# syghmon/bridges-with-reinforcement-learning

Measured on AMD Instinct MI355X. Metric: env-steps/sec (vectorised assembly_gym, tower_height=4), higher is better.
Workload: dtype f64

## Files before the change

bridges-with-reinforcement-learning_amd/csrc/api.hip:

```cpp
#include <hip/hip_runtime.h>
#include <cstdio>
#include <cstdlib>
#include <cstring>
#include <new>

#include "env_kernels.hip"
#include "ops_kernels.hip"
#include "dqn_kernels.hip"
#include "mlp_kernels.hip"
#include "conv_kernels.hip"
#include "conv_train_kernels.hip"

using namespace bridges;

static thread_local char g_err[512] = "";

static int fail_hip(hipError_t e, const char* what) {
    snprintf(g_err, sizeof(g_err), "%s: %s", what, hipGetErrorString(e));
    return BRIDGES_E_HIP;
}
static int fail_arg(const char* what) {
    snprintf(g_err, sizeof(g_err), "bad argument: %s", what);
    return BRIDGES_E_ARG;
}
#define HIP_TRY(x)                                        \
    do {                                                  \
        hipError_t e_ = (x);                              \
        if (e_ != hipSuccess) return fail_hip(e_, #x);    \
    } while (0)

template <typename... P, typename... A>
static int launch(const char* name, void (*k)(P...), dim3 grid, dim3 block, size_t lds, void* stream, A... a) {
    hipLaunchKernelGGL(k, grid, block, lds, (hipStream_t)stream, a...);
    const hipError_t e = hipGetLastError();
    return e == hipSuccess ? BRIDGES_OK : fail_hip(e, name);
}

template <typename... T>
static bool aligned(uintptr_t bytes, const T*... p) {
    return ((((uintptr_t)p) | ... | (uintptr_t)0) & (bytes - 1)) == 0;
}

static int64_t ceil_div(int64_t a, int64_t b) { return (a + b - 1) / b; }

static int64_t clamp_grid(int64_t blocks, int64_t limit) {
    if (blocks < 1) blocks = 1;
    return blocks > limit ? limit : blocks;
}

static int grid_for_waves(int64_t n_items) { return (int)clamp_grid(ceil_div(n_items, 4), 2048); }

static int up2_splits(int64_t tiles, int* tps) {
    int per = (int)((tiles + 255) / 256);
    if (per < 1) per = 1;
    *tps = per;
    return (int)((tiles + per - 1) / per);
}

typedef void (*c3_fn)(const float*, const float*, const float*, const float*, const float*, float*, int, int, int, int, int);
template <int W, int CH>
static c3_fn c3_epilogue(int mode) {
    if (mode == C3_EPI_BIAS_RELU) return k_c3<W, CH, C3_EPI_BIAS_RELU>;
    if (mode == C3_EPI_MASK) return k_c3<W, CH, C3_EPI_MASK>;
    return k_c3<W, CH, C3_EPI_RAW>;
}
template <int W>
static c3_fn c3_kernel(int c_in, int mode) { return c_in <= 4 ? c3_epilogue<W, 4>(mode) : c3_epilogue<W, 16>(mode); }

struct bridges_gate {
    hipEvent_t last;
};

struct bridges_env {
    bridges_gate* gate;
    hipEvent_t raster_done;
    DevCtx ctx;
    TaskTable* tt_dev;
    int32_t* h_total;
    int max_blocks;
    int max_faces;
    hipEvent_t* ev_start;
    hipEvent_t* ev_stop;
    int ev_cap, ev_used;
    bool has_tasks;
    bridges_task_buffers tasks;
    const float* fixed_reward_map;
    const double* fixed_reward_prefix;
};

static long long candidate_estimate(const bridges_env* env) {
    long long est = (long long)(*(volatile int32_t*)env->h_total);
    if (est < env->ctx.E) est = env->ctx.E;
    return est + est / 32 + 64;
}

extern "C" {

const char* bridges_last_error(void) { return g_err; }

#ifndef BRIDGES_SRC_HASH
#define BRIDGES_SRC_HASH "unstamped"
#endif
const char* bridges_source_hash(void) { return "BRIDGES_SRC_HASH=" BRIDGES_SRC_HASH; }

int bridges_device_count(void) {
    int n = 0;
    if (hipGetDeviceCount(&n) != hipSuccess) return 0;
    return n;
}

int bridges_env_create(const bridges_task* t, const bridges_env_buffers* buf, bridges_env** out) {
    if (!t || !buf || !out) return fail_arg("null");
    if (t->n_envs <= 0) return fail_arg("n_envs");
    if (t->max_blocks <= 0 || t->max_blocks > BRIDGES_MAX_BLOCKS) return fail_arg("max_blocks > BRIDGES_MAX_BLOCKS");
    if (t->n_shapes <= 0 || t->n_shapes > 8) return fail_arg("n_shapes");
    if (t->n_groups <= 0 || t->n_groups > BRIDGES_MAX_GROUPS) return fail_arg("n_groups");
    if (t->n_ground < 0 || t->n_ground > 32 || t->n_offsets <= 0 || t->n_offsets > 8) return fail_arg("n_ground/n_offsets");
    if (t->n_targets < 0 || t->n_targets > BRIDGES_MAX_TARGETS) return fail_arg("n_targets");
    if (t->a_max <= 0) return fail_arg("a_max");
    if (t->img_size != 0 && (t->img_size < 2 || t->img_size > BRIDGES_IMG)) return fail_arg("img_size must be 0 (= 64) or 2..64");
    if (t->debug != 0) return fail_arg("debug must be 0");
    if (!buf->reward_prefix) return fail_arg("reward_prefix (float64 row prefix sums of reward_map) not given");
    if (buf->lp_ws_stride < (int64_t)BRIDGES_LP_WS_DOUBLES) return fail_arg("lp_ws_stride < BRIDGES_LP_WS_DOUBLES");
    static_assert(BRIDGES_LP_WS_DOUBLES == WARM_WS_DOUBLES, "header and device code disagree on the persistent tableau size");
    static_assert(BRIDGES_LP_SNAP_DOUBLES == WARM_HDR_DOUBLES + WARM_HALF, "header and device code disagree on the snapshot size");
    if (buf->lp_snap && buf->lp_snap_stride < (int64_t)BRIDGES_LP_SNAP_DOUBLES) return fail_arg("lp_snap_stride < BRIDGES_LP_SNAP_DOUBLES");
    for (int g = 0; g < t->n_groups; ++g) {
        if (t->group_shape[g] < 0 || t->group_shape[g] >= t->n_shapes) return fail_arg("group_shape");
        if (t->group_face[g] < 0 || t->group_face[g] >= t->shapes[t->group_shape[g]].nv) return fail_arg("group_face");
    }
    for (int s = 0; s < t->n_shapes; ++s)
        if (t->shapes[s].nv < 3 || t->shapes[s].nv > BRIDGES_MAX_VERTS) return fail_arg("shape nv");
    int ndev = 0;
    if (hipGetDeviceCount(&ndev) != hipSuccess || ndev == 0) {
        snprintf(g_err, sizeof(g_err), "no HIP device");
        return BRIDGES_E_NODEV;
    }
    bridges_env* env = new (std::nothrow) bridges_env();
    if (!env) return fail_arg("oom");
    TaskTable* host = new (std::nothrow) TaskTable();
    if (!host) { delete env; return fail_arg("oom"); }
    memset(host, 0, sizeof(TaskTable));
    memcpy(host->shapes, t->shapes, sizeof(bridges_shape) * t->n_shapes);
    memcpy(host->x_ground, t->x_ground, sizeof(double) * t->n_ground);
    memcpy(host->offsets, t->offsets, sizeof(double) * t->n_offsets);
    const int img = t->img_size ? t->img_size : IMG;
    for (int i = 0; i < IMG; ++i) {
        host->grid_x[i] = t->grid_x[i < img ? i : img - 1];
        host->grid_y[i] = t->grid_y[i < img ? i : img - 1];
    }
    hipError_t e = hipMalloc((void**)&env->tt_dev, sizeof(TaskTable));
    if (e == hipSuccess) e = hipMemcpy(env->tt_dev, host, sizeof(TaskTable), hipMemcpyHostToDevice);
    delete host;
    if (e != hipSuccess) { delete env; return fail_hip(e, "task table upload"); }
    DevCtx& c = env->ctx;
    memset(&c, 0, sizeof(c));
    c.b = *buf;
    c.tt = env->tt_dev;
    c.E = t->n_envs; c.K = t->max_blocks; c.max_steps = t->max_steps; c.a_max = t->a_max;
    c.n_groups = t->n_groups; c.n_ground = t->n_ground; c.n_offsets = t->n_offsets; c.n_targets = t->n_targets;
    memcpy(c.group_shape, t->group_shape, sizeof(c.group_shape));
    memcpy(c.group_face, t->group_face, sizeof(c.group_face));
    c.mu = t->mu; c.density = t->density; c.floor_hw = t->floor_half_width; c.floor_depth = t->floor_depth;
    c.xlim0 = t->xlim[0]; c.xlim1 = t->xlim[1]; c.ylim0 = t->ylim[0]; c.ylim1 = t->ylim[1];
    memcpy(c.targets, t->targets, sizeof(c.targets));
    c.seed = t->seed;
    c.debug = t->debug;
    c.env_id_base = t->env_id_base;
    c.n_shapes = t->n_shapes;
    c.img = img;
    env->ev_start = env->ev_stop = nullptr;
    env->ev_cap = env->ev_used = 0;
    env->gate = nullptr;
    env->raster_done = nullptr;
    env->has_tasks = false;
    memset(&env->tasks, 0, sizeof(env->tasks));
// ... 20 lines not shown
    }
    delete[] env->ev_start;
    delete[] env->ev_stop;
    env->ev_start = env->ev_stop = nullptr;
    env->ev_cap = env->ev_used = 0;
}

int bridges_env_destroy(bridges_env* env) {
    if (!env) return BRIDGES_OK;
    free_events(env);
    if (env->raster_done) (void)hipEventDestroy(env->raster_done);
    (void)hipFree(env->tt_dev);
    (void)hipHostFree(env->h_total);
    delete env;
    return BRIDGES_OK;
}

int bridges_gate_create(bridges_gate** out) {
    if (!out) return fail_arg("gate_create");
    bridges_gate* g = new (std::nothrow) bridges_gate();
    if (!g) return fail_arg("oom");
    g->last = nullptr;
    *out = g;
    return BRIDGES_OK;
}

int bridges_gate_destroy(bridges_gate* gate) {
    delete gate;
    return BRIDGES_OK;
}

int bridges_env_set_gate(bridges_env* env, bridges_gate* gate) {
    if (!env) return fail_arg("set_gate");
    if (gate && !env->raster_done) HIP_TRY(hipEventCreateWithFlags(&env->raster_done, hipEventDisableTiming));
    env->gate = gate;
    return BRIDGES_OK;
}

int bridges_env_timing_begin(bridges_env* env, int32_t max_launches) {
    if (!env || max_launches <= 0 || max_launches > (1 << 16)) return fail_arg("timing_begin");
    free_events(env);
    env->ev_start = new (std::nothrow) hipEvent_t[max_launches];
    env->ev_stop = new (std::nothrow) hipEvent_t[max_launches];
    if (!env->ev_start || !env->ev_stop) {
        delete[] env->ev_start;
        delete[] env->ev_stop;
        env->ev_start = env->ev_stop = nullptr;
        return fail_arg("oom");
    }
    for (int i = 0; i < max_launches; ++i) {
        HIP_TRY(hipEventCreate(&env->ev_start[i]));
        HIP_TRY(hipEventCreate(&env->ev_stop[i]));
        env->ev_cap = i + 1;
    }
    env->ev_used = 0;
    return BRIDGES_OK;
}

int bridges_env_timing_end(bridges_env* env, double* raster_ms_total, int32_t* n_launches) {
    if (!env || !raster_ms_total || !n_launches) return fail_arg("timing_end");
    double total = 0.0;
    for (int i = 0; i < env->ev_used; ++i) {
        HIP_TRY(hipEventSynchronize(env->ev_stop[i]));
        float ms = 0.f;
        HIP_TRY(hipEventElapsedTime(&ms, env->ev_start[i], env->ev_stop[i]));
        total += ms;
    }
    *raster_ms_total = total;
    *n_launches = env->ev_used;
    free_events(env);
    return BRIDGES_OK;
}

static int refresh(bridges_env* env, hipStream_t s, int after_step) {
    const DevCtx& c = env->ctx;
    if (int rc = launch("k_scan", k_scan, dim3(1), dim3(SCAN_THREADS), 0, s, c, after_step)) return rc;
    if (int rc = launch("k_enumerate", k_enumerate, dim3(c.E), dim3(WAVE), 0, s, c)) return rc;
    const long long items_est = candidate_estimate(env) + c.E;
    long long rblocks = ceil_div(items_est, 4);
    if (rblocks > env->max_blocks) rblocks = env->max_blocks;
    const bool timed = env->ev_cap > 0 && env->ev_used < env->ev_cap;
    if (env->gate && env->gate->last) HIP_TRY(hipStreamWaitEvent(s, env->gate->last, 0));
    if (timed) HIP_TRY(hipEventRecord(env->ev_start[env->ev_used], s));
    if (!env->has_tasks) {
        if (int rc = launch("k_raster", env->max_faces <= 4 ? k_raster<4> : k_raster<MAXV>, dim3((unsigned)rblocks), dim3(256), 0, s, c))
            return rc;
    } else if (int rc = launch("k_raster (per-env tables)", env->max_faces <= 4 ? k_raster<4, true> : k_raster<MAXV, true>,
                               dim3((unsigned)rblocks), dim3(256), 0, s, c)) {
        return rc;
    }
    if (timed) { HIP_TRY(hipEventRecord(env->ev_stop[env->ev_used], s)); env->ev_used++; }
    if (env->gate) {
        HIP_TRY(hipEventRecord(env->raster_done, s));
        env->gate->last = env->raster_done;
    }
    return launch("k_select", k_select, dim3(c.E), dim3(WAVE), 0, s, c, 0);
}

static int task_features(bridges_env* env, void* stream, int mode) {
    return launch("k_task_features", k_task_features, dim3(env->ctx.E), dim3(TASK_THREADS), 0, stream, env->ctx, env->tasks, mode);
}

int bridges_env_reset(bridges_env* env, void* stream) {
    if (!env) return fail_arg("null env");
    if (int rc = launch("k_reset", k_reset, dim3(env->ctx.E), dim3(WAVE), 0, stream, env->ctx)) return rc;
    if (env->has_tasks)
        if (int rc = task_features(env, stream, TASK_RESET)) return rc;
    return refresh(env, (hipStream_t)stream, 0);
}

int bridges_env_step(bridges_env* env, void* stream) {
    if (!env) return fail_arg("null env");
    if (!env->has_tasks) {
        if (int rc = launch("k_step", k_step<>, dim3(env->ctx.E), dim3(WAVE), 0, stream, env->ctx)) return rc;
    } else {
        if (int rc = launch("k_step (per-env targets)", k_step<const double*>, dim3(env->ctx.E), dim3(WAVE), 0, stream, env->ctx,
                            (const double*)env->tasks.env_targets))
            return rc;
        if (env->tasks.sample)
            if (int rc = task_features(env, stream, TASK_STEP)) return rc;
    }
    return refresh(env, (hipStream_t)stream, 1);
}

int bridges_env_set_task_buffers(bridges_env* env, const bridges_task_buffers* tb) {
    if (!env) return fail_arg("null env");
    DevCtx& c = env->ctx;
    if (!tb) {
        env->has_tasks = false;
        memset(&env->tasks, 0, sizeof(env->tasks));
        c.b.reward_map = env->fixed_reward_map;
        c.b.reward_prefix = env->fixed_reward_prefix;
        return BRIDGES_OK;
    }
    if (!tb->env_targets || !tb->target_bits || !tb->reward_map || !tb->reward_prefix || !tb->task_episode || !tb->gauss_k)
        return fail_arg("task buffers: env_targets / target_bits / reward_map / reward_prefix / task_episode / gauss_k not given");
    if (tb->env_obstacle_bits) return fail_arg("task buffers: env_obstacle_bits is reserved (obstacles are shared by all envs)");
    if (c.n_targets < 1) return fail_arg("task buffers: the task has no targets");
    if (tb->target_shape < 0 || tb->target_shape >= c.n_shapes) return fail_arg("task buffers: target_shape");
    if (tb->sample != 0 && tb->sample != 1) return fail_arg("task buffers: sample must be 0 or 1");
    if (tb->sample && !(tb->x_range[0] <= tb->x_range[1] && tb->z_range[0] <= tb->z_range[1])) return fail_arg("task buffers: x_range / z_range");
    env->tasks = *tb;
    env->has_tasks = true;
    c.b.reward_map = tb->reward_map;
    c.b.reward_prefix = tb->reward_prefix;
    return BRIDGES_OK;
}

int bridges_env_load_targets(bridges_env* env, void* stream) {
    if (!env) return fail_arg("null env");
    if (!env->has_tasks) return fail_arg("bridges_env_load_targets: no task buffers attached");
    return task_features(env, stream, TASK_LOAD);
}

int bridges_env_refresh(bridges_env* env, void* stream) {
    if (!env) return fail_arg("null env");
    return refresh(env, (hipStream_t)stream, 0);
}

#define CS_TAB_SMALL 768
#define CS_COLS_SMALL 92
#define CS_TAB_LARGE 4096
int bridges_env_candidate_stability(bridges_env* env, void* stream) {
    if (!env) return fail_arg("null env");
    const DevCtx& c = env->ctx;
    if (!c.b.cand_stable || !c.b.cand_queue || !c.b.cand_counters || !c.b.cand_ws) return fail_arg("cand_stable / cand_queue / cand_counters / cand_ws not given");
    if (c.b.cand_ws_stride < (int64_t)(3 * c.K + 2) * (4 * BRIDGES_MAX_INTERFACES + 3)) return fail_arg("cand_ws_stride");
    hipStream_t s = (hipStream_t)stream;
    HIP_TRY(hipMemsetAsync(c.b.cand_counters, 0, 2 * sizeof(int32_t), s));
    long long est = candidate_estimate(env);
    if (est > env->max_blocks) est = env->max_blocks;
    if (int rc = launch("k_candidate_stability", k_candidate_stability<CS_TAB_SMALL, CS_COLS_SMALL, false>, dim3((unsigned)est),
                        dim3(WAVE), 0, s, c))
// ... 820 lines not shown
```

bridges-with-reinforcement-learning_amd/csrc/env_kernels.hip:

```cpp
#include "bridges_device.h"
#include "rbe_device.h"

namespace bridges {

__device__ inline void reset_env(const DevCtx& c, int e, int lane) {
    c.b.state_bits[(size_t)e * IMG + lane] = 0ull;
    if (lane < c.K) c.b.blk_occ[(size_t)e * c.K + lane] = 0;
    if (lane == 0) {
        c.b.n_blocks[e] = 0;
        c.b.n_if[e] = 0;
        c.b.targets_left[e] = (c.n_targets >= 32) ? 0xffffffffu : ((1u << c.n_targets) - 1u);
        c.b.needs_reset[e] = 0;
    }
}

__device__ inline int count_candidates(const DevCtx& c, int e, int nb, int lane) {
    int nfree = 0;
    for (int i0 = 0; i0 < nb * MAXV; i0 += WAVE) {
        int i = i0 + lane;
        bool fr = false;
        if (i < nb * MAXV) {
            int b = i / MAXV, f = i % MAXV;
            int nv = c.tt->shapes[c.b.blk_shape[(size_t)e * c.K + b]].nv;
            fr = f < nv && !((c.b.blk_occ[(size_t)e * c.K + b] >> f) & 1);
// ... 426 lines not shown
                rot2(sn.vx[i], sn.vz[i], cs, sn_, rx, rz);
                wx[i] = px + rx; wz[i] = pz + rz;
                if (wx[i] < c.xlim0 - eps || wx[i] > c.xlim1 + eps || wz[i] < c.ylim0 - eps || wz[i] > c.ylim1 + eps) inb = false;
                if (wz[i] < -eps) inb = false;
            }
            c.b.cand_verts[ci * MAXV * 2 + 2 * i] = wx[i];
            c.b.cand_verts[ci * MAXV * 2 + 2 * i + 1] = wz[i];
        }
        {
#define PICK6(v, k) ((k) == 5 ? v[5] : (k) == 4 ? v[4] : (k) == 3 ? v[3] : (k) == 2 ? v[2] : (k) == 1 ? v[1] : v[0])
#pragma unroll
            for (int f = 0; f < MAXV; ++f) {
                double o0 = 0.0, o1 = 0.0, o2 = 0.0, o3 = 0.0;
                if (f < sn.nv) {
                    const int ia = sn.fa[f], ib = sn.fb[f];
                    const double ax = PICK6(wx, ia), az = PICK6(wz, ia), bx = PICK6(wx, ib), bz = PICK6(wz, ib);
                    Frame2 fr = edge_frame(ax, az, bx, bz);
                    o0 = fr.cx; o1 = fr.cz; o2 = fr.nx; o3 = fr.nz;
                }
                double2* dst = reinterpret_cast<double2*>(c.b.cand_frames + (ci * MAXV + f) * 4);
                dst[0] = make_double2(o0, o1);
                dst[1] = make_double2(o2, o3);
            }
#undef PICK6
            c.b.cand_rows[ci * 2 + 0] = (sn.nv << 16) | ((inb ? 1 : 0) << 24);
            c.b.cand_rows[ci * 2 + 1] = e;
        }
        c.b.cand_pose[ci * 4 + 0] = px; c.b.cand_pose[ci * 4 + 1] = pz;
        c.b.cand_pose[ci * 4 + 2] = cs; c.b.cand_pose[ci * 4 + 3] = sn_;
        c.b.cand_desc[ci * 4 + 0] = tb; c.b.cand_desc[ci * 4 + 1] = tf;
        c.b.cand_desc[ci * 4 + 2] = sh; c.b.cand_desc[ci * 4 + 3] = fc;
        c.b.cand_ox[ci] = ox;
        c.b.cand_inb[ci] = inb;
        c.b.cand_env[ci] = e;
    }
}

__device__ __forceinline__ void write_f32_image(float* img, uint64_t rowbits, int lane, int32_t* nz = nullptr) {
    const int sub = lane >> 4, col4 = (lane & 15) * 4;
    const uint64_t nonzero_rows = __ballot(rowbits != 0ull);
    if (nz) {
        uint64_t t = nonzero_rows | (nonzero_rows >> 1);
        t = (t | (t >> 2)) & 0x1111111111111111ull;
        uint32_t now = 0u;
#pragma unroll
        for (int g = 0; g < IMG / 4; ++g) now |= (uint32_t)((t >> (4 * g)) & 1ull) << g;
        uint32_t need = (uint32_t)__builtin_amdgcn_readfirstlane(*nz) | now;
        if (lane == 0) *nz = (int32_t)now;
        while (need) {
            const int g = __builtin_ctz(need);
            need &= need - 1u;
            uint32_t nib = 0u;
            if ((now >> g) & 1u) {
                uint64_t m = shfl_u64(rowbits, 4 * g + sub);
                nib = (uint32_t)(m >> col4) & 0xFu;
            }
            float4 v;
            v.x = (nib & 1u) ? 1.f : 0.f;
            v.y = (nib & 2u) ? 1.f : 0.f;
            v.z = (nib & 4u) ? 1.f : 0.f;
            v.w = (nib & 8u) ? 1.f : 0.f;
            *reinterpret_cast<float4*>(img + (size_t)(4 * g + sub) * IMG + col4) = v;
        }
        return;
    }
#pragma unroll
    for (int r0 = 0; r0 < IMG; r0 += 4) {
        uint32_t nib = 0u;
        if ((nonzero_rows >> r0) & 0xFull) {
            uint64_t m = shfl_u64(rowbits, r0 + sub);
            nib = (uint32_t)(m >> col4) & 0xFu;
        }
        float4 v;
        v.x = (nib & 1u) ? 1.f : 0.f;
        v.y = (nib & 2u) ? 1.f : 0.f;
        v.z = (nib & 4u) ? 1.f : 0.f;
        v.w = (nib & 8u) ? 1.f : 0.f;
        *reinterpret_cast<float4*>(img + (size_t)(r0 + sub) * IMG + col4) = v;
    }
}

__device__ __forceinline__ uint64_t low_mask64(int n) { return n >= 64 ? ~0ull : ((1ull << n) - 1ull); }

template <int NF, int F0 = 0>
__device__ __forceinline__ uint64_t raster_rows(double fr0, double fr1, double fr2, double fr3, int n_img, double X, double Y,
                                                int lane) {
    int alo[NF], ahi[NF], pos[NF];
    double t[NF];
    bool rev[NF];
#pragma unroll
    for (int f = 0; f < NF; ++f) {
        const double cxf = readlane_d(fr0, F0 + f), czf = readlane_d(fr1, F0 + f), nxf = readlane_d(fr2, F0 + f), nzf = readlane_d(fr3, F0 + f);
        const double a = (X - cxf) * nxf;
        t[f] = -((Y - czf) * nzf);
        alo[f] = __double2loint(a);
        ahi[f] = __double2hiint(a);
        rev[f] = nxf < 0.0;
        pos[f] = 0;
    }
#define RASTER_PROBE(S_, INC_)                                                                                          \
    _Pragma("unroll") for (int f = 0; f < NF; ++f) {                                                                    \
        const int j = pos[f] + (S_);                                                                                    \
        const int src = rev[f] ? 63 - j : j;                                                                            \
        const double av = __hiloint2double(__shfl(ahi[f], src, WAVE), __shfl(alo[f], src, WAVE));                       \
        if (av <= t[f]) pos[f] += (INC_);                                                                               \
    }
    RASTER_PROBE(31, 32) RASTER_PROBE(15, 16) RASTER_PROBE(7, 8) RASTER_PROBE(3, 4) RASTER_PROBE(1, 2) RASTER_PROBE(0, 1)
    RASTER_PROBE(0, 1)
#undef RASTER_PROBE
    uint64_t bits = low_mask64(n_img);
#pragma unroll
    for (int f = 0; f < NF; ++f) {
        const uint64_t run = low_mask64(pos[f]);
        bits &= rev[f] ? (pos[f] ? ~low_mask64(64 - pos[f]) : 0ull) : run;
    }
    return lane < n_img ? bits : 0ull;
}

__device__ __forceinline__ uint64_t raster_rows6(double fr0, double fr1, double fr2, double fr3, int n_img, double X, double Y, int lane) {
    return raster_rows<3, 0>(fr0, fr1, fr2, fr3, n_img, X, Y, lane) & raster_rows<3, 3>(fr0, fr1, fr2, fr3, n_img, X, Y, lane);
}

__device__ __forceinline__ uint64_t raster_rows_nv(double fr0, double fr1, double fr2, double fr3, int nv, int n_img, double X,
                                                   double Y, int lane) {
    return nv <= 4 ? raster_rows<4>(fr0, fr1, fr2, fr3, n_img, X, Y, lane) : raster_rows6(fr0, fr1, fr2, fr3, n_img, X, Y, lane);
}

__device__ __forceinline__ void raster_reward_fetch(uint64_t rowbits, const double* prefix, int lane, double& p_hi, double& p_lo) {
    p_hi = 0.0; p_lo = 0.0;
    if (rowbits) {
        const int lo = __builtin_ctzll(rowbits), hi = 64 - __builtin_clzll(rowbits);
        const double* p = prefix + lane * (IMG + 1);
        p_hi = p[hi]; p_lo = p[lo];
    }
}
__device__ __forceinline__ double raster_reward_sum(double p_hi, double p_lo) { return wave_sum_d(p_hi - p_lo); }

__device__ __forceinline__ uint64_t raster_outline(const double* v , int nv, const int32_t* fa,
                                                   const int32_t* fb, const double* gx, const double* gy, int size, int lane) {
    double cx = 0.0, cz = 0.0, nx = 0.0, nz = 0.0;
    if (lane < nv) {
        Frame2 fr = edge_frame(v[2 * fa[lane]], v[2 * fa[lane] + 1], v[2 * fb[lane]], v[2 * fb[lane] + 1]);
        cx = fr.cx; cz = fr.cz; nx = fr.nx; nz = fr.nz;
    }
    const int g = lane < size ? lane : size - 1;
    return raster_rows_nv(cx, cz, nx, nz, nv, size, gx[g], gy[g], lane);
}

template <int NF, bool PER_ENV = false>
__global__ __launch_bounds__(256) void k_raster(DevCtx c) {
    const int lane = threadIdx.x & (WAVE - 1);
    const int wave = (blockIdx.x * blockDim.x + threadIdx.x) / WAVE;
    const int nwaves = (gridDim.x * blockDim.x) / WAVE;
    const int total = c.b.cand_offset[c.E];
    const int items = total + (c.b.state_raster ? c.E : 0);
    const double X = c.tt->grid_x[lane], Y = c.tt->grid_y[lane];
    const uint64_t obst = c.b.obstacle_bits[lane];
    for (int itv = wave; itv < items; itv += nwaves) {
        const int it = __builtin_amdgcn_readfirstlane(itv);
        if (it < total) {
            const size_t ci = (size_t)it;
            const int meta = c.b.cand_rows[ci * 2];
            const int e = c.b.cand_rows[ci * 2 + 1];
            const int nv = (meta >> 16) & 0xff;
            const bool inb = (meta >> 24) & 1;
            (void)nv;
            double fr0 = 0.0, fr1 = 0.0, fr2 = 0.0, fr3 = 0.0;
            if (lane < MAXV) {
                const double2* p = reinterpret_cast<const double2*>(c.b.cand_frames + (ci * MAXV + lane) * 4);
                const double2 a = p[0], b = p[1];
                fr0 = a.x; fr1 = a.y; fr2 = b.x; fr3 = b.y;
            }
            const uint64_t occ = c.b.state_bits[(size_t)e * IMG + lane] | obst;
            const uint64_t bits = (NF == 4 || nv <= 4) ? raster_rows<4>(fr0, fr1, fr2, fr3, c.img, X, Y, lane)
                                                       : raster_rows6(fr0, fr1, fr2, fr3, c.img, X, Y, lane);
            const bool overlap = __ballot((bits & occ) != 0ull) != 0ull;
            double p_hi, p_lo;
            raster_reward_fetch(bits, PER_ENV ? c.b.reward_prefix + (size_t)e * (IMG * (IMG + 1)) : c.b.reward_prefix, lane, p_hi, p_lo);
            c.b.cand_bits[ci * IMG + lane] = bits;
            if (c.b.cand_raster)
                write_f32_image(c.b.cand_raster + ci * IMG * IMG, bits, lane, c.b.cand_raster_nz ? c.b.cand_raster_nz + ci : nullptr);
            const double lin = raster_reward_sum(p_hi, p_lo);
            if (lane == 0) {
                c.b.cand_lin[ci] = (float)lin;
                c.b.cand_mask[ci] = (uint8_t)(inb && !overlap);
            }
        } else {
            const int e = it - total;
            write_f32_image(c.b.state_raster + (size_t)e * IMG * IMG, c.b.state_bits[(size_t)e * IMG + lane], lane,
                            c.b.state_raster_nz ? c.b.state_raster_nz + e : nullptr);
        }
    }
}


enum { TASK_LOAD = 0, TASK_RESET = 1, TASK_STEP = 2 };
#define TASK_SALT 0x7461736B5F726E67ull
#define TASK_ROW (IMG + 1)
#define TASK_WAVES 4
#define TASK_THREADS (TASK_WAVES * WAVE)
#define TASK_ROWS_IN_FLIGHT 4
#define TASK_KZ_PAD 16
#define TASK_KZ (TASK_KZ_PAD + BRIDGES_GAUSS_TAPS + 16)
static_assert(IMG - 1 - BRIDGES_GAUSS_TAPS / 2 <= TASK_KZ_PAD && IMG - 1 + BRIDGES_GAUSS_TAPS / 2 < BRIDGES_GAUSS_TAPS + 16,
              "every tap index of a 64 x 64 canvas must fall into the padded table");
static_assert(IMG % (TASK_WAVES * TASK_ROWS_IN_FLIGHT) == 0, "map rows are dealt to the waves in batches");
__global__ __launch_bounds__(TASK_THREADS) void k_task_features(DevCtx c, bridges_task_buffers t, int mode) {
    __shared__ float kz[TASK_KZ];
    __shared__ uint64_t tb_l[IMG];
    __shared__ double tv_l[TASK_WAVES][MAXV * 2];
    __shared__ float map_l[IMG * TASK_ROW];
    __shared__ double pre_l[IMG * TASK_ROW];
    const int e = blockIdx.x, tid = threadIdx.x, lane = tid & (WAVE - 1), wv = tid / WAVE;
    const int T = c.n_targets, S = c.img;
    if (mode == TASK_STEP) {
        const uint8_t* fl = c.b.step_flags + (size_t)e * 8;
        if (fl[F_VALID] && !fl[F_DONE]) return;
    }
    for (int i = tid; i < TASK_KZ; i += TASK_THREADS) {
        const int tap = i - TASK_KZ_PAD;
        kz[i] = (tap >= 0 && tap < BRIDGES_GAUSS_TAPS) ? t.gauss_k[tap] : 0.f;
    }
    double* tg = t.env_targets + (size_t)e * T * 3;
    uint32_t ep = 0u;
    if (mode == TASK_STEP) ep = t.task_episode[e] + 1u;
    __syncthreads();
    if (mode != TASK_LOAD && tid == 0) t.task_episode[e] = ep;
    double tv = 0.0;
    if (lane < 3 * T) {
        if (t.sample && mode != TASK_LOAD) {
            const int axis = lane % 3;
            if (axis != 1) {
                const uint64_t h0 = splitmix64((((c.seed & 0xFFFFFFFFull) << 32) | (uint32_t)(c.env_id_base + e)) ^ TASK_SALT);
                const uint64_t h1 = splitmix64(h0 ^ (uint64_t)ep);
                const uint64_t r = splitmix64(h1 ^ (uint64_t)lane);
                const double u = (double)(r >> 11) * 0x1.0p-53;
                const double lo = axis == 0 ? t.x_range[0] : t.z_range[0], hi = axis == 0 ? t.x_range[1] : t.z_range[1];
                const double span = hi - lo;
                const double step = span * u;
                tv = lo + step;
            }
            if (wv == 0) tg[lane] = tv;
        } else {
            tv = tg[lane];
        }
    }
    const bridges_shape& cube = c.tt->shapes[t.target_shape];
    const int nv = cube.nv;
    uint64_t bits = 0ull;
    for (int q = 0; q < T; ++q) {
        const double px = readlane_d(tv, 3 * q), pz = readlane_d(tv, 3 * q + 2);
        __syncthreads();
        if (lane < nv) { tv_l[wv][2 * lane] = px + cube.vx[lane]; tv_l[wv][2 * lane + 1] = pz + cube.vz[lane]; }
        __syncthreads();
        bits |= raster_outline(tv_l[wv], nv, cube.fa, cube.fb, c.tt->grid_x, c.tt->grid_y, S, lane);
    }
    if (wv == 0) {
        tb_l[lane] = bits;
        t.target_bits[(size_t)e * IMG + lane] = bits;
    }
    __syncthreads();
    const uint64_t nzrows = __ballot(bits != 0ull);
    const int half = BRIDGES_GAUSS_TAPS / 2;
    float* map_g = t.reward_map + (size_t)e * IMG * IMG;
    for (int b = 0; b < IMG / (TASK_WAVES * TASK_ROWS_IN_FLIGHT); ++b) {
        const int y0 = (wv * (IMG / TASK_WAVES)) + b * TASK_ROWS_IN_FLIGHT;
        double acc[TASK_ROWS_IN_FLIGHT];
#pragma unroll
        for (int r = 0; r < TASK_ROWS_IN_FLIGHT; ++r) acc[r] = 0.0;
        uint64_t rows = y0 < S ? nzrows : 0ull;
        while (rows) {
            const int py = __builtin_ctzll(rows);
            rows &= rows - 1ull;
            float ki[TASK_ROWS_IN_FLIGHT];
#pragma unroll
// ... 272 lines not shown
```

bridges-with-reinforcement-learning_amd/csrc/bridges_device.h:

```cpp
#pragma once
#include <hip/hip_runtime.h>
#include <stdint.h>
#include "../../include/bridges_hip.h"

#define WAVE 64
#define MAXV BRIDGES_MAX_VERTS
#define MAXK BRIDGES_MAX_BLOCKS
#define MAXIF BRIDGES_MAX_INTERFACES
#define IMG BRIDGES_IMG

namespace bridges {

struct Frame2 {
    double cx, cz, tx, tz, nx, nz;
};

__device__ __forceinline__ Frame2 edge_frame(double ax, double az, double bx, double bz) {
    Frame2 f;
    f.cx = (ax + bx) * 0.5;
    f.cz = (az + bz) * 0.5;
    double dx = bx - ax;
    double dz = bz - az;
    double L = sqrt(dx * dx + dz * dz);
    f.tx = dx / L;
    f.tz = dz / L;
    f.nx = -f.tz;
    f.nz = f.tx;
    return f;
}

__device__ __forceinline__ void rot2(double vx, double vz, double c, double s, double& ox, double& oz) {
    ox = vx * c + vz * s;
    oz = vz * c - vx * s;
}

__device__ __forceinline__ void align_place(const Frame2& f1, double c2x, double c2z, double n2x, double n2z,
                                            double ox, double oy, double& px, double& pz, double& c, double& s) {
    double dot = f1.nx * n2x + f1.nz * n2z;
    c = -dot;
    if (c > 1.0) c = 1.0;
    if (c < -1.0) c = -1.0;
    double cy = f1.nz * n2x - f1.nx * n2z;
    s = (cy + 1e-6 >= 0) ? fabs(cy) : -fabs(cy);
    double r2x, r2z;
    rot2(c2x, c2z, c, s, r2x, r2z);
    px = ((f1.cx + ox * f1.tx) + oy * f1.nx) - r2x;
    pz = ((f1.cz + ox * f1.tz) + oy * f1.nz) - r2z;
}

__device__ __forceinline__ uint64_t splitmix64(uint64_t x) {
    x += 0x9E3779B97F4A7C15ull;
    uint64_t z = x;
    z = (z ^ (z >> 30)) * 0xBF58476D1CE4E5B9ull;
    z = (z ^ (z >> 27)) * 0x94D049BB133111EBull;
    return z ^ (z >> 31);
}

__device__ __forceinline__ float relu_nan(float v) { return v <= 0.f ? 0.f : v; }
__device__ __forceinline__ float max_nan(float a, float b) { return (b > a || b != b) ? b : a; }
__device__ __forceinline__ float max4_nan(float a, float b, float c, float d) { return max_nan(max_nan(a, b), max_nan(c, d)); }

__device__ __forceinline__ double shfl_d(double v, int src) { return __shfl(v, src, WAVE); }

__device__ __forceinline__ uint64_t shfl_u64(uint64_t v, int src) {
    uint32_t lo = (uint32_t)v, hi = (uint32_t)(v >> 32);
    lo = __shfl(lo, src, WAVE);
    hi = __shfl(hi, src, WAVE);
    return ((uint64_t)hi << 32) | lo;
}

#define DPP_QUAD_XOR1 0xB1
#define DPP_QUAD_XOR2 0x4E
#define DPP_ROW_HALF_MIRROR 0x141
#define DPP_ROW_MIRROR 0x140
#define DPP_ROW_BCAST15 0x142
#define DPP_ROW_BCAST31 0x143

template <int CTRL, int ROW_MASK>
__device__ __forceinline__ int dpp_i(int old, int x) {
    return __builtin_amdgcn_update_dpp(old, x, CTRL, ROW_MASK, 0xF, false);
}
template <int CTRL, int ROW_MASK>
__device__ __forceinline__ double dpp_d(double old, double x) {
    int lo = dpp_i<CTRL, ROW_MASK>(__double2loint(old), __double2loint(x));
    int hi = dpp_i<CTRL, ROW_MASK>(__double2hiint(old), __double2hiint(x));
    return __hiloint2double(hi, lo);
}
__device__ __forceinline__ double readlane_d(double v, int lane_uniform) {
    int lo = __builtin_amdgcn_readlane(__double2loint(v), lane_uniform);
    int hi = __builtin_amdgcn_readlane(__double2hiint(v), lane_uniform);
    return __hiloint2double(hi, lo);
}
#define WAVE_REDUCE_D(OP, IDENT_OLD)                                                   \
    v = OP(v, dpp_d<DPP_QUAD_XOR1, 0xF>(v, v));                                        \
    v = OP(v, dpp_d<DPP_QUAD_XOR2, 0xF>(v, v));                                        \
    v = OP(v, dpp_d<DPP_ROW_HALF_MIRROR, 0xF>(v, v));                                  \
    v = OP(v, dpp_d<DPP_ROW_MIRROR, 0xF>(v, v));                                       \
    v = OP(v, dpp_d<DPP_ROW_BCAST15, 0xA>(IDENT_OLD, v));                              \
    v = OP(v, dpp_d<DPP_ROW_BCAST31, 0xC>(IDENT_OLD, v));                              \
    return readlane_d(v, 63);

__device__ __forceinline__ double add_d_(double a, double b) { return a + b; }
__device__ __forceinline__ double min_raw_d(double a, double b) { double r; asm volatile("v_min_f64 %0, %1, %2\n\ts_nop 1" : "=v"(r) : "v"(a), "v"(b)); return r; }
__device__ __forceinline__ double max_raw_d(double a, double b) { double r; asm volatile("v_max_f64 %0, %1, %2\n\ts_nop 1" : "=v"(r) : "v"(a), "v"(b)); return r; }
__device__ __forceinline__ double wave_sum_d(double v) { WAVE_REDUCE_D(add_d_, 0.0) }
__device__ __forceinline__ double wave_min_d(double v) { WAVE_REDUCE_D(min_raw_d, v) }
__device__ __forceinline__ double wave_max_d(double v) { WAVE_REDUCE_D(max_raw_d, v) }
__device__ __forceinline__ int wave_min_i(int v) {
    v = min(v, dpp_i<DPP_QUAD_XOR1, 0xF>(v, v));
    v = min(v, dpp_i<DPP_QUAD_XOR2, 0xF>(v, v));
    v = min(v, dpp_i<DPP_ROW_HALF_MIRROR, 0xF>(v, v));
    v = min(v, dpp_i<DPP_ROW_MIRROR, 0xF>(v, v));
    v = min(v, dpp_i<DPP_ROW_BCAST15, 0xA>(v, v));
    v = min(v, dpp_i<DPP_ROW_BCAST31, 0xC>(v, v));
    return __builtin_amdgcn_readlane(v, 63);
}

struct TaskTable {
    bridges_shape shapes[8];
    double x_ground[32];
    double offsets[8];
    double grid_x[IMG];
    double grid_y[IMG];
};

struct DevCtx {
    bridges_env_buffers b;
    const TaskTable* tt;
    int32_t* h_total;
    int32_t E, K, max_steps, a_max, n_groups, n_ground, n_offsets, n_targets;
    int32_t debug, env_id_base;
    int32_t n_shapes, img;
    int32_t group_shape[BRIDGES_MAX_GROUPS];
    int32_t group_face[BRIDGES_MAX_GROUPS];
    double mu, density, floor_hw, floor_depth;
    double xlim0, xlim1, ylim0, ylim1;
    double targets[BRIDGES_MAX_TARGETS][3];
    uint64_t seed;
};

enum { F_VALID = 0, F_STABLE_FROZEN, F_STABLE_UNFROZEN, F_TERMINATED, F_TRUNCATED, F_DONE, F_NO_ACTIONS, F_LP_ERROR };
enum { ST_SUM_CAND = 0, ST_SUM_BLOCKS, ST_ENV_STEPS, ST_RESET_ONLY, ST_LP_ERRORS, ST_IF_OVERFLOW, ST_LOCKSTEPS, ST_SUM_VALID, ST_WARM_RESOLVED, ST_CAND_OVERFLOW };

// ... 2 lines not shown
```

Baseline: 4.915 million.

## Prefetch raster candidate metadata and specialize kernel for full raster writes

The raster kernel now loads each candidate's row metadata and edge frames through a helper, issuing the first load before the loop and the next one at the end of each iteration. This is meant to hide global-memory latency. A FULL template variant drops the nonzero-count pointer checks when dense rasters are written without nz tracking, and the kernel gains a waves_per_eu hint. The overlap test moves after the stores, and the grid and obstacle loads use wavefront-scoped relaxed atomic loads. The trade-offs are extra template instantiations and possible register pressure from the occupancy hint.

After: 4.966 million, median of 4. +1.0%, better.

```diff
diff --git a/bridges-with-reinforcement-learning_amd/csrc/api.hip b/bridges-with-reinforcement-learning_amd/csrc/api.hip
--- a/bridges-with-reinforcement-learning_amd/csrc/api.hip
+++ b/bridges-with-reinforcement-learning_amd/csrc/api.hip
@@ -278,12 +278,14 @@
     const bool timed = env->ev_cap > 0 && env->ev_used < env->ev_cap;
     if (env->gate && env->gate->last) HIP_TRY(hipStreamWaitEvent(s, env->gate->last, 0));
     if (timed) HIP_TRY(hipEventRecord(env->ev_start[env->ev_used], s));
+    const bool full = c.b.cand_raster && !c.b.cand_raster_nz;
+    const bool four = env->max_faces <= 4;
     if (!env->has_tasks) {
-        if (int rc = launch("k_raster", env->max_faces <= 4 ? k_raster<4> : k_raster<MAXV>, dim3((unsigned)rblocks), dim3(256), 0, s, c))
-            return rc;
-    } else if (int rc = launch("k_raster (per-env tables)", env->max_faces <= 4 ? k_raster<4, true> : k_raster<MAXV, true>,
-                               dim3((unsigned)rblocks), dim3(256), 0, s, c)) {
-        return rc;
+        auto k = full ? (four ? k_raster<4, false, true> : k_raster<MAXV, false, true>) : (four ? k_raster<4> : k_raster<MAXV>);
+        if (int rc = launch("k_raster", k, dim3((unsigned)rblocks), dim3(RASTER_THREADS), 0, s, c)) return rc;
+    } else {
+        auto k = full ? (four ? k_raster<4, true, true> : k_raster<MAXV, true, true>) : (four ? k_raster<4, true> : k_raster<MAXV, true>);
+        if (int rc = launch("k_raster (per-env tables)", k, dim3((unsigned)rblocks), dim3(RASTER_THREADS), 0, s, c)) return rc;
     }
     if (timed) { HIP_TRY(hipEventRecord(env->ev_stop[env->ev_used], s)); env->ev_used++; }
     if (env->gate) {
diff --git a/bridges-with-reinforcement-learning_amd/csrc/env_kernels.hip b/bridges-with-reinforcement-learning_amd/csrc/env_kernels.hip
--- a/bridges-with-reinforcement-learning_amd/csrc/env_kernels.hip
+++ b/bridges-with-reinforcement-learning_amd/csrc/env_kernels.hip
@@ -597,39 +597,57 @@
     return raster_rows_nv(cx, cz, nx, nz, nv, size, gx[g], gy[g], lane);
 }
 
-template <int NF, bool PER_ENV = false>
-__global__ __launch_bounds__(256) void k_raster(DevCtx c) {
+constexpr int RASTER_THREADS = 256;
+
+struct RasterRequest { int row; double fr0, fr1, fr2, fr3; };
+__device__ __forceinline__ RasterRequest raster_request(const DevCtx& c, int it, int last_slot, int lane) {
+    const size_t ci = (size_t)(it < last_slot ? it : last_slot);
+    const int32_t* rows = c.b.cand_rows + ci * 2;
+    const double2* frames = reinterpret_cast<const double2*>(c.b.cand_frames + ci * (MAXV * 4));
+    RasterRequest q;
+    q.row = rows[(unsigned)lane & 1u];
+    q.fr0 = 0.0; q.fr1 = 0.0; q.fr2 = 0.0; q.fr3 = 0.0;
+    if (lane < MAXV) {
+        const double2 a = frames[(unsigned)lane * 2u], b = frames[(unsigned)lane * 2u + 1u];
+        q.fr0 = a.x; q.fr1 = a.y; q.fr2 = b.x; q.fr3 = b.y;
+    }
+    return q;
+}
+
+template <typename T>
+__device__ __forceinline__ T load_here(const T* p) { return __hip_atomic_load(p, __ATOMIC_RELAXED, __HIP_MEMORY_SCOPE_WAVEFRONT); }
+
+template <int NF, bool PER_ENV = false, bool FULL = false>
+__global__ __launch_bounds__(RASTER_THREADS) __attribute__((amdgpu_waves_per_eu(8))) void k_raster(DevCtx c) {
     const int lane = threadIdx.x & (WAVE - 1);
-    const int wave = (blockIdx.x * blockDim.x + threadIdx.x) / WAVE;
-    const int nwaves = (gridDim.x * blockDim.x) / WAVE;
+    const int wave = blockIdx.x * (RASTER_THREADS / WAVE) + threadIdx.x / WAVE;
+    const int nwaves = gridDim.x * (RASTER_THREADS / WAVE);
+    const int last_slot = c.E * c.a_max - 1;
+    int it = __builtin_amdgcn_readfirstlane(wave);
+    RasterRequest q = raster_request(c, it, last_slot, lane);
+    const double X = load_here(c.tt->grid_x + lane), Y = load_here(c.tt->grid_y + lane);
+    const uint64_t obst = load_here(c.b.obstacle_bits + lane);
     const int total = c.b.cand_offset[c.E];
     const int items = total + (c.b.state_raster ? c.E : 0);
-    const double X = c.tt->grid_x[lane], Y = c.tt->grid_y[lane];
-    const uint64_t obst = c.b.obstacle_bits[lane];
-    for (int itv = wave; itv < items; itv += nwaves) {
-        const int it = __builtin_amdgcn_readfirstlane(itv);
+    while (it < items) {
         if (it < total) {
             const size_t ci = (size_t)it;
-            const int meta = c.b.cand_rows[ci * 2];
-            const int e = c.b.cand_rows[ci * 2 + 1];
+            const int meta = __builtin_amdgcn_readlane(q.row, 0);
+            const int e = __builtin_amdgcn_readlane(q.row, 1);
             const int nv = (meta >> 16) & 0xff;
-            const bool inb = (meta >> 24) & 1;
             (void)nv;
-            double fr0 = 0.0, fr1 = 0.0, fr2 = 0.0, fr3 = 0.0;
-            if (lane < MAXV) {
-                const double2* p = reinterpret_cast<const double2*>(c.b.cand_frames + (ci * MAXV + lane) * 4);
-                const double2 a = p[0], b = p[1];
-                fr0 = a.x; fr1 = a.y; fr2 = b.x; fr3 = b.y;
-            }
-            const uint64_t occ = c.b.state_bits[(size_t)e * IMG + lane] | obst;
-            const uint64_t bits = (NF == 4 || nv <= 4) ? raster_rows<4>(fr0, fr1, fr2, fr3, c.img, X, Y, lane)
-                                                       : raster_rows6(fr0, fr1, fr2, fr3, c.img, X, Y, lane);
-            const bool overlap = __ballot((bits & occ) != 0ull) != 0ull;
+            const uint64_t srow = (c.b.state_bits + (size_t)e * IMG)[(unsigned)lane];
+            const uint64_t bits = (NF == 4 || nv <= 4) ? raster_rows<4>(q.fr0, q.fr1, q.fr2, q.fr3, c.img, X, Y, lane)
+                                                       : raster_rows6(q.fr0, q.fr1, q.fr2, q.fr3, c.img, X, Y, lane);
             double p_hi, p_lo;
             raster_reward_fetch(bits, PER_ENV ? c.b.reward_prefix + (size_t)e * (IMG * (IMG + 1)) : c.b.reward_prefix, lane, p_hi, p_lo);
-            c.b.cand_bits[ci * IMG + lane] = bits;
-            if (c.b.cand_raster)
+            (c.b.cand_bits + ci * IMG)[(unsigned)lane] = bits;
+            if (FULL)
+                write_f32_image(c.b.cand_raster + ci * IMG * IMG, bits, lane);
+            else if (c.b.cand_raster)
                 write_f32_image(c.b.cand_raster + ci * IMG * IMG, bits, lane, c.b.cand_raster_nz ? c.b.cand_raster_nz + ci : nullptr);
+            const bool overlap = __ballot((bits & (srow | obst)) != 0ull) != 0ull;
+            const bool inb = (meta >> 24) & 1;
             const double lin = raster_reward_sum(p_hi, p_lo);
             if (lane == 0) {
                 c.b.cand_lin[ci] = (float)lin;
@@ -640,6 +658,9 @@
             write_f32_image(c.b.state_raster + (size_t)e * IMG * IMG, c.b.state_bits[(size_t)e * IMG + lane], lane,
                             c.b.state_raster_nz ? c.b.state_raster_nz + e : nullptr);
         }
+        it += nwaves;
+        if (it >= items) break;
+        q = raster_request(c, it, last_slot, lane);
     }
 }
 
```

## Load raster candidate frames via scalar constant loads and specialize raster modes

Applied to the files above, without the earlier changes.

The raster kernel now fetches each candidate's metadata and edge frames through constant-address-space pointers, so they land in scalar registers. This replaces the per-lane vector loads followed by readlane broadcasts. Frames are loaded before the bounds check, using a clamped row index, and inline asm pins them to SGPRs. Output mode (bits only, f32 image, sparse) becomes a template parameter chosen on the host, and waves-per-EU hints and sched barriers are added. The reward prefix fetch also becomes branchless. This cuts VALU and readlane work and branching per candidate, at the cost of more SGPR pressure and relying on a row clamp for safe speculative loads.

Measured after the change: 4.957 million before, 4.426 million after. 10.7% lower.

```diff
diff --git a/bridges-with-reinforcement-learning_amd/csrc/api.hip b/bridges-with-reinforcement-learning_amd/csrc/api.hip
--- a/bridges-with-reinforcement-learning_amd/csrc/api.hip
+++ b/bridges-with-reinforcement-learning_amd/csrc/api.hip
@@ -92,6 +92,18 @@
     long long est = (long long)(*(volatile int32_t*)env->h_total);
     if (est < env->ctx.E) est = env->ctx.E;
     return est + est / 32 + 64;
+}
+
+typedef void (*raster_kernel_t)(DevCtx);
+template <int NF, bool PER_ENV>
+static raster_kernel_t raster_kernel_mode(const bridges_env_buffers& b) {
+    if (!b.cand_raster) return k_raster<NF, PER_ENV, RASTER_BITS>;
+    return b.cand_raster_nz ? k_raster<NF, PER_ENV, RASTER_SPARSE> : k_raster<NF, PER_ENV, RASTER_F32>;
+}
+static raster_kernel_t raster_kernel(const bridges_env* env) {
+    const bridges_env_buffers& b = env->ctx.b;
+    if (env->max_faces <= 4) return env->has_tasks ? raster_kernel_mode<4, true>(b) : raster_kernel_mode<4, false>(b);
+    return env->has_tasks ? raster_kernel_mode<MAXV, true>(b) : raster_kernel_mode<MAXV, false>(b);
 }
 
 extern "C" {
@@ -278,13 +290,8 @@
     const bool timed = env->ev_cap > 0 && env->ev_used < env->ev_cap;
     if (env->gate && env->gate->last) HIP_TRY(hipStreamWaitEvent(s, env->gate->last, 0));
     if (timed) HIP_TRY(hipEventRecord(env->ev_start[env->ev_used], s));
-    if (!env->has_tasks) {
-        if (int rc = launch("k_raster", env->max_faces <= 4 ? k_raster<4> : k_raster<MAXV>, dim3((unsigned)rblocks), dim3(256), 0, s, c))
-            return rc;
-    } else if (int rc = launch("k_raster (per-env tables)", env->max_faces <= 4 ? k_raster<4, true> : k_raster<MAXV, true>,
-                               dim3((unsigned)rblocks), dim3(256), 0, s, c)) {
+    if (int rc = launch(env->has_tasks ? "k_raster (per-env tables)" : "k_raster", raster_kernel(env), dim3((unsigned)rblocks), dim3(256), 0, s, c))
         return rc;
-    }
     if (timed) { HIP_TRY(hipEventRecord(env->ev_stop[env->ev_used], s)); env->ev_used++; }
     if (env->gate) {
         HIP_TRY(hipEventRecord(env->raster_done, s));
diff --git a/bridges-with-reinforcement-learning_amd/csrc/bridges_device.h b/bridges-with-reinforcement-learning_amd/csrc/bridges_device.h
--- a/bridges-with-reinforcement-learning_amd/csrc/bridges_device.h
+++ b/bridges-with-reinforcement-learning_amd/csrc/bridges_device.h
@@ -59,6 +59,12 @@
 __device__ __forceinline__ float relu_nan(float v) { return v <= 0.f ? 0.f : v; }
 __device__ __forceinline__ float max_nan(float a, float b) { return (b > a || b != b) ? b : a; }
 __device__ __forceinline__ float max4_nan(float a, float b, float c, float d) { return max_nan(max_nan(a, b), max_nan(c, d)); }
+
+#define BRIDGES_CONSTANT_AS __attribute__((address_space(4)))
+template <typename T>
+__device__ __forceinline__ const BRIDGES_CONSTANT_AS T* scalar_ptr(const T* p) {
+    return (const BRIDGES_CONSTANT_AS T*)p;
+}
 
 __device__ __forceinline__ double shfl_d(double v, int src) { return __shfl(v, src, WAVE); }
 
diff --git a/bridges-with-reinforcement-learning_amd/csrc/env_kernels.hip b/bridges-with-reinforcement-learning_amd/csrc/env_kernels.hip
--- a/bridges-with-reinforcement-learning_amd/csrc/env_kernels.hip
+++ b/bridges-with-reinforcement-learning_amd/csrc/env_kernels.hip
@@ -532,15 +532,14 @@
 
 __device__ __forceinline__ uint64_t low_mask64(int n) { return n >= 64 ? ~0ull : ((1ull << n) - 1ull); }
 
-template <int NF, int F0 = 0>
-__device__ __forceinline__ uint64_t raster_rows(double fr0, double fr1, double fr2, double fr3, int n_img, double X, double Y,
-                                                int lane) {
+template <int NF>
+__device__ __forceinline__ uint64_t raster_rows_uniform(const double* fr , int n_img, double X, double Y, int lane) {
     int alo[NF], ahi[NF], pos[NF];
     double t[NF];
     bool rev[NF];
 #pragma unroll
     for (int f = 0; f < NF; ++f) {
-        const double cxf = readlane_d(fr0, F0 + f), czf = readlane_d(fr1, F0 + f), nxf = readlane_d(fr2, F0 + f), nzf = readlane_d(fr3, F0 + f);
+        const double cxf = fr[4 * f], czf = fr[4 * f + 1], nxf = fr[4 * f + 2], nzf = fr[4 * f + 3];
         const double a = (X - cxf) * nxf;
         t[f] = -((Y - czf) * nzf);
         alo[f] = __double2loint(a);
@@ -567,6 +566,18 @@
     return lane < n_img ? bits : 0ull;
 }
 
+template <int NF, int F0 = 0>
+__device__ __forceinline__ uint64_t raster_rows(double fr0, double fr1, double fr2, double fr3, int n_img, double X, double Y,
+                                                int lane) {
+    double fr[4 * NF];
+#pragma unroll
+    for (int f = 0; f < NF; ++f) {
+        fr[4 * f] = readlane_d(fr0, F0 + f); fr[4 * f + 1] = readlane_d(fr1, F0 + f);
+        fr[4 * f + 2] = readlane_d(fr2, F0 + f); fr[4 * f + 3] = readlane_d(fr3, F0 + f);
+    }
+    return raster_rows_uniform<NF>(fr, n_img, X, Y, lane);
+}
+
 __device__ __forceinline__ uint64_t raster_rows6(double fr0, double fr1, double fr2, double fr3, int n_img, double X, double Y, int lane) {
     return raster_rows<3, 0>(fr0, fr1, fr2, fr3, n_img, X, Y, lane) & raster_rows<3, 3>(fr0, fr1, fr2, fr3, n_img, X, Y, lane);
 }
@@ -577,12 +588,9 @@
 }
 
 __device__ __forceinline__ void raster_reward_fetch(uint64_t rowbits, const double* prefix, int lane, double& p_hi, double& p_lo) {
-    p_hi = 0.0; p_lo = 0.0;
-    if (rowbits) {
-        const int lo = __builtin_ctzll(rowbits), hi = 64 - __builtin_clzll(rowbits);
-        const double* p = prefix + lane * (IMG + 1);
-        p_hi = p[hi]; p_lo = p[lo];
-    }
+    const int lo = rowbits ? __builtin_ctzll(rowbits) : 0, hi = rowbits ? 64 - __builtin_clzll(rowbits) : 0;
+    const double* p = prefix + lane * (IMG + 1);
+    p_hi = p[hi]; p_lo = p[lo];
 }
 __device__ __forceinline__ double raster_reward_sum(double p_hi, double p_lo) { return wave_sum_d(p_hi - p_lo); }
 
@@ -597,50 +605,83 @@
     return raster_rows_nv(cx, cz, nx, nz, nv, size, gx[g], gy[g], lane);
 }
 
-template <int NF, bool PER_ENV = false>
-__global__ __launch_bounds__(256) void k_raster(DevCtx c) {
+enum { RASTER_F32 = 0, RASTER_SPARSE = 1, RASTER_BITS = 2 };
+
+__device__ __forceinline__ void pin_scalar_loads(int meta, int e, const double* fr ) {
+    asm volatile("" ::"s"(meta), "s"(e), "s"(fr[0]), "s"(fr[1]), "s"(fr[2]), "s"(fr[3]), "s"(fr[4]), "s"(fr[5]), "s"(fr[6]), "s"(fr[7]),
+                 "s"(fr[8]), "s"(fr[9]), "s"(fr[10]), "s"(fr[11]));
+}
+__device__ __forceinline__ void pin_scalar_loads(const double* fr ) {
+    asm volatile("" ::"s"(fr[0]), "s"(fr[1]), "s"(fr[2]), "s"(fr[3]));
+}
+
+template <int NF, bool PER_ENV, int MODE>
+__device__ __forceinline__ bool raster_item(const DevCtx& c, int it, int total, int items, int last_row, int lane, double X, double Y,
+                                            uint64_t obst) {
+    const size_t row = (size_t)min(it, last_row);
+    const BRIDGES_CONSTANT_AS int32_t* rp = scalar_ptr(c.b.cand_rows) + row * 2;
+    const BRIDGES_CONSTANT_AS double* fp = scalar_ptr(c.b.cand_frames) + row * (MAXV * 4);
+    const int meta = rp[0], e_cand = rp[1];
+    constexpr int NF0 = NF == 4 ? 4 : 3;
+    double fr[4 * NF0];
+#pragma unroll
+    for (int k = 0; k < 4 * NF0; ++k) fr[k] = fp[k];
+    pin_scalar_loads(meta, e_cand, fr);
+    if (NF == 4) pin_scalar_loads(fr + 12);
+    if (it >= items) return false;
+    if (it < total) {
+        const size_t ci = (size_t)it;
+        const int e = e_cand;
+        const uint64_t state = c.b.state_bits[(size_t)e * IMG + lane];
+        __builtin_amdgcn_sched_barrier(0);
+        const int nv = (meta >> 16) & 0xff;
+        const bool inb = (meta >> 24) & 1;
+        uint64_t bits;
+        if (NF == 4) {
+            bits = raster_rows_uniform<NF0>(fr, c.img, X, Y, lane);
+        } else {
+            double fr1[12];
+#pragma unroll
+            for (int k = 0; k < 12; ++k) fr1[k] = fp[12 + k];
+            if (nv <= 4) {
+                const double f4[16] = {fr[0], fr[1], fr[2], fr[3], fr[4], fr[5], fr[6], fr[7], fr[8], fr[9], fr[10], fr[11],
+                                       fr1[0], fr1[1], fr1[2], fr1[3]};
+                bits = raster_rows_uniform<4>(f4, c.img, X, Y, lane);
+            } else {
+                bits = raster_rows_uniform<3>(fr, c.img, X, Y, lane) & raster_rows_uniform<3>(fr1, c.img, X, Y, lane);
+            }
+        }
+        double p_hi, p_lo;
+        raster_reward_fetch(bits, PER_ENV ? c.b.reward_prefix + (size_t)e * (IMG * (IMG + 1)) : c.b.reward_prefix, lane, p_hi, p_lo);
+        c.b.cand_bits[ci * IMG + lane] = bits;
+        if (MODE == RASTER_F32) write_f32_image(c.b.cand_raster + ci * IMG * IMG, bits, lane);
+        if (MODE == RASTER_SPARSE) write_f32_image(c.b.cand_raster + ci * IMG * IMG, bits, lane, c.b.cand_raster_nz + ci);
+        __builtin_amdgcn_sched_barrier(0);
+        const double lin = raster_reward_sum(p_hi, p_lo);
+        const bool overlap = __ballot((bits & (state | obst)) != 0ull) != 0ull;
+        if (lane == 0) {
+            c.b.cand_lin[ci] = (float)lin;
+            c.b.cand_mask[ci] = (uint8_t)(inb && !overlap);
+        }
+    } else {
+        const int e = it - total;
+        write_f32_image(c.b.state_raster + (size_t)e * IMG * IMG, c.b.state_bits[(size_t)e * IMG + lane], lane,
+                        c.b.state_raster_nz ? c.b.state_raster_nz + e : nullptr);
+    }
+    return true;
+}
+
+template <int NF, bool PER_ENV = false, int MODE = RASTER_F32>
+__global__ __launch_bounds__(256) __attribute__((amdgpu_waves_per_eu(NF > 4 && MODE == RASTER_F32 ? 8 : 1, 8))) void k_raster(DevCtx c) {
     const int lane = threadIdx.x & (WAVE - 1);
-    const int wave = (blockIdx.x * blockDim.x + threadIdx.x) / WAVE;
-    const int nwaves = (gridDim.x * blockDim.x) / WAVE;
-    const int total = c.b.cand_offset[c.E];
-    const int items = total + (c.b.state_raster ? c.E : 0);
     const double X = c.tt->grid_x[lane], Y = c.tt->grid_y[lane];
     const uint64_t obst = c.b.obstacle_bits[lane];
-    for (int itv = wave; itv < items; itv += nwaves) {
-        const int it = __builtin_amdgcn_readfirstlane(itv);
-        if (it < total) {
-            const size_t ci = (size_t)it;
-            const int meta = c.b.cand_rows[ci * 2];
-            const int e = c.b.cand_rows[ci * 2 + 1];
-            const int nv = (meta >> 16) & 0xff;
-            const bool inb = (meta >> 24) & 1;
-            (void)nv;
-            double fr0 = 0.0, fr1 = 0.0, fr2 = 0.0, fr3 = 0.0;
-            if (lane < MAXV) {
-                const double2* p = reinterpret_cast<const double2*>(c.b.cand_frames + (ci * MAXV + lane) * 4);
-                const double2 a = p[0], b = p[1];
-                fr0 = a.x; fr1 = a.y; fr2 = b.x; fr3 = b.y;
-            }
-            const uint64_t occ = c.b.state_bits[(size_t)e * IMG + lane] | obst;
-            const uint64_t bits = (NF == 4 || nv <= 4) ? raster_rows<4>(fr0, fr1, fr2, fr3, c.img, X, Y, lane)
-                                                       : raster_rows6(fr0, fr1, fr2, fr3, c.img, X, Y, lane);
-            const bool overlap = __ballot((bits & occ) != 0ull) != 0ull;
-            double p_hi, p_lo;
-            raster_reward_fetch(bits, PER_ENV ? c.b.reward_prefix + (size_t)e * (IMG * (IMG + 1)) : c.b.reward_prefix, lane, p_hi, p_lo);
-            c.b.cand_bits[ci * IMG + lane] = bits;
-            if (c.b.cand_raster)
-                write_f32_image(c.b.cand_raster + ci * IMG * IMG, bits, lane, c.b.cand_raster_nz ? c.b.cand_raster_nz + ci : nullptr);
-            const double lin = raster_reward_sum(p_hi, p_lo);
-            if (lane == 0) {
-                c.b.cand_lin[ci] = (float)lin;
-                c.b.cand_mask[ci] = (uint8_t)(inb && !overlap);
-            }
-        } else {
-            const int e = it - total;
-            write_f32_image(c.b.state_raster + (size_t)e * IMG * IMG, c.b.state_bits[(size_t)e * IMG + lane], lane,
-                            c.b.state_raster_nz ? c.b.state_raster_nz + e : nullptr);
-        }
-    }
+    const int wave = (int)blockIdx.x * (256 / WAVE) + __builtin_amdgcn_readfirstlane((int)threadIdx.x / WAVE);
+    const int nwaves = (int)gridDim.x * (256 / WAVE);
+    const int last_row = c.E * c.a_max - 1;
+    const int total = scalar_ptr(c.b.cand_offset)[c.E];
+    const int items = total + (c.b.state_raster ? c.E : 0);
+    for (int it = wave; raster_item<NF, PER_ENV, MODE>(c, it, total, items, last_row, lane, X, Y, obst); it += nwaves) {}
 }
 
 
```
